# double125/MADTP

Hardware: AMD Instinct MI355X
Metric: images/sec forward, BLIP-base NLVR2 p=0.5 b64; pruned-token index match (higher is better)
Workload: dtype bf16

## Files before the change

madtp_amd/csrc/gemm_device.h:

```cpp
#pragma once
#include "common.h"
#include <type_traits>

namespace {


constexpr int ROWB = 128;
constexpr int NTHREADS = 256;

struct GemmArgs {
    const char* A; const char* W; const float* bias; const float* residual; void* C;
    int M, N, K, lda, ldw, ldc, ldr, act, ntm, ntn, dbg, fast_epi, splitk, ngrp;
    const char* A2; const char* W2; const float* bias2; void* C2; int pair;
    float out_scale;
    float acc_scale;
    float acc_scale2;
    float* sk_ws; int* sk_tick; int sk;
    int desc;
    int* range_flag;
    const int32_t* m_dev; int m_mul;
};
struct F16P { unsigned short bits; };

struct F16S {};
__device__ __forceinline__ bf16x8 x3_scale_lo(bf16x8 q) {
    const f16x8 v = __builtin_bit_cast(f16x8, q) * (_Float16)(1.0f / F16S_LO_SCALE);
    return __builtin_bit_cast(bf16x8, v);
}
template <bool F16>
__device__ __forceinline__ f32x4 mfma_16x16x32(bf16x8 a, bf16x8 b, f32x4 c) {
    if constexpr (F16)
        return __builtin_amdgcn_mfma_f32_16x16x32_f16(__builtin_bit_cast(f16x8, a), __builtin_bit_cast(f16x8, b), c, 0, 0, 0);
    else
        return __builtin_amdgcn_mfma_f32_16x16x32_bf16(a, b, c, 0, 0, 0);
}
constexpr int OM_F32 = 0, OM_BF16 = 1, OM_F16S = 2, OM_F16 = 3;

__device__ __forceinline__ float apply_act(float v, int act) {
    switch (act) {
        case MADTP_ACT_GELU_ERF: return 0.5f * v * (1.0f + erff(v * 0.70710678118654752440f));
        case MADTP_ACT_QUICK_GELU: return v / (1.0f + expf(-1.702f * v));
        case MADTP_ACT_RELU: return fmaxf(v, 0.0f);
        default: return v;
    }
}

template <bool PERM>
__device__ __forceinline__ int swz_key(int r) { return PERM ? (((r >> 1) & 1) | (((r >> 3) & 3) << 1)) : (r & 7); }

__device__ __forceinline__ void xcd_tiles(int T, int xcd, int& t0, int& nt) {
    t0 = (int)(((long)xcd * T) >> 3);
    nt = (int)(((long)(xcd + 1) * T) >> 3) - t0;
}

__device__ __forceinline__ void tile_mn(const GemmArgs& g, int t, int& tm, int& tn) {
    if (g.ngrp == 0) { tm = t / g.ntn; tn = t % g.ntn; return; }
    const int per = g.ntm * g.ngrp;
    const int grp = t / per, r = t - grp * per;
    const int gw = min(g.ngrp, g.ntn - grp * g.ngrp);
    tm = r / gw; tn = grp * g.ngrp + (r - tm * gw);
}

template <int NQ>
__device__ __forceinline__ void stage_tile_desc(const char* base, unsigned bytes, const unsigned* roff, int soff, char* lds) {
    const __amdgpu_buffer_rsrc_t rs = __builtin_amdgcn_make_buffer_rsrc((void*)base, 0, bytes, 0x00020000);
#pragma unroll
    for (int q = 0; q < NQ; ++q) __builtin_amdgcn_raw_ptr_buffer_load_lds(rs, LDS_PTR(lds + q * 1024), 16, roff[q], soff, 0, 0);
}

template <int ESZ, int ROWS, bool PERM = false>
__device__ __forceinline__ void stage_tile(const char* base, int row0, int max_row, int ld_elems, int kbyte0,
                                           char* lds_tile, int wave, int lane, int tile_row0 = 0) {
    const int sub = lane >> 3;
#pragma unroll
    for (int q = 0; q < ROWS / 32; ++q) {
        const int grp = wave * (ROWS / 32) + q;
        const int chunk = (lane & 7) ^ swz_key<PERM>(tile_row0 + grp * 8 + sub);
        int row = row0 + grp * 8 + sub;
        row = row < max_row ? row : max_row;
        const char* src = base + ((size_t)row * ld_elems) * ESZ + kbyte0 + chunk * 16;
        __builtin_amdgcn_global_load_lds(GLOBAL_PTR(src), LDS_PTR(lds_tile + grp * 1024), 16, 0, 0);
    }
}

template <int N> __device__ __forceinline__ void wait_vmcnt() { asm volatile("s_waitcnt vmcnt(%0)" ::"n"(N) : "memory"); }

__device__ __forceinline__ float gelu_fast(float v) {
    constexpr float L2E = 1.4426950408889634f;
    const float x2 = fminf(v * v, 25.0f);
    float p = fmaf(x2, 7.03033581e-04f * L2E, -7.40112921e-02f * L2E);
    p = fmaf(x2, p, -1.59501577f * L2E);
    const float e = __builtin_amdgcn_exp2f(v * p);
    return v * __builtin_amdgcn_rcpf(1.0f + e);
}

template <bool LP_OUT, int ACT>
__device__ __forceinline__ float epi_act(float v) {
    if constexpr (ACT == MADTP_ACT_GELU_ERF) return LP_OUT ? gelu_fast(v) : 0.5f * v * (1.0f + erff(v * 0.70710678118654752440f));
    else if constexpr (ACT == MADTP_ACT_QUICK_GELU)
        return LP_OUT ? v * __builtin_amdgcn_rcpf(1.0f + __builtin_amdgcn_exp2f(-1.702f * 1.4426950408889634f * v))
                      : v / (1.0f + expf(-1.702f * v));
    else if constexpr (ACT == MADTP_ACT_RELU) return fmaxf(v, 0.0f);
    else return v;
}

template <bool LP_OUT>
__host__ __device__ __forceinline__ constexpr int wfrag_row(int j, int rho) {
    return LP_OUT ? 32 * (j >> 1) + 8 * (rho >> 2) + 4 * (j & 1) + (rho & 3) : 16 * j + rho;
}

template <int OM, int ACT, bool HAS_RES, int FM, int FN, int BM, int BN, bool FAST_ONLY = false, int RM = 1, int RN = 1>
__device__ __forceinline__ void epilogue(const GemmArgs& g, const f32x4 (&acc)[FM][FN], const f32x4 (&res)[RM][RN],
                                         int m0, int n0, int wr, int wc, int l16, int grp4, size_t c_off) {
    constexpr bool LP_OUT = OM != OM_F32;
    constexpr bool FAST_ACT = OM == OM_BF16 || OM == OM_F16;
    const bool c_bf16 = g.ldc < 0;
    const int ldc = c_bf16 ? -g.ldc : g.ldc;
            const int col_w = n0 + wc * (BN / 2);
            if (FAST_ONLY || g.fast_epi) {
                constexpr int NJ = LP_OUT ? FN / 2 : FN;
                constexpr int NV = LP_OUT ? 2 : 1;
                constexpr int CSZ = LP_OUT ? 2 : 4;
                constexpr bool RES_PREF = !LP_OUT && RM == FM;
                float range_mx = 0.f;
                const int row_t = m0 + wr * (BM / 2);
                const int rows_valid = max(min(g.M - row_t, BM / 2), 0);
                const unsigned long long cb = (unsigned long long)((char*)g.C + (c_off + (size_t)((g.dbg & 8) ? (row_t & 127) : row_t) * ldc) * CSZ);
                const unsigned cb_lo = __builtin_amdgcn_readfirstlane((unsigned)cb);
                const unsigned cb_hi = __builtin_amdgcn_readfirstlane((unsigned)(cb >> 32));
                const __amdgpu_buffer_rsrc_t crsrc = __builtin_amdgcn_make_buffer_rsrc(
                    (void*)(((unsigned long long)cb_hi << 32) | cb_lo), 0,
                    __builtin_amdgcn_readfirstlane(rows_valid * ldc * CSZ), 0x00020000);
                int colv[NJ];
                bool cok[NJ];
                f32x4 bv[NJ][NV];
#pragma unroll
                for (int jv = 0; jv < NJ; ++jv) {
                    colv[jv] = col_w + (LP_OUT ? 32 * jv + 8 * grp4 : 16 * jv + 4 * grp4);
                    cok[jv] = colv[jv] < g.N;
#pragma unroll
                    for (int u = 0; u < NV; ++u) bv[jv][u] = (f32x4){0.f, 0.f, 0.f, 0.f};
                }
                if (g.bias) {
#pragma unroll
                    for (int jv = 0; jv < NJ; ++jv)
#pragma unroll
                        for (int u = 0; u < NV; ++u) bv[jv][u] = *(const f32x4*)(g.bias + (cok[jv] ? colv[jv] : 0) + 4 * u);
                }
                constexpr bool RES_LOAD = HAS_RES && !RES_PREF;
                constexpr int IC = RES_LOAD ? (FM > 2 ? FM / 2 : FM) : FM;
                f32x4 rv[RES_LOAD ? IC : 1][RES_LOAD ? NJ : 1][NV];
#pragma unroll
                for (int i0 = 0; i0 < FM; i0 += IC) {
                    if constexpr (RES_LOAD) {
#pragma unroll
                        for (int ii = 0; ii < IC; ++ii) {
                            const int row = min(row_t + l16 + 16 * (i0 + ii), g.M - 1);
#pragma unroll
                            for (int jv = 0; jv < NJ; ++jv) {
                                const float* rp = g.residual + (size_t)row * g.ldr + (cok[jv] ? colv[jv] : 0);
#pragma unroll
                                for (int u = 0; u < NV; ++u) rv[ii][jv][u] = *(const f32x4*)(rp + 4 * u);
                            }
                        }
                    }
                    if (RES_LOAD || i0 == 0) {
                        __builtin_amdgcn_sched_barrier(0);
                        __builtin_amdgcn_s_waitcnt(0x0F70);
                        __builtin_amdgcn_sched_barrier(0);
                    }
#pragma unroll
                    for (int ii = 0; ii < IC; ++ii) {
                        const int i = i0 + ii;
#pragma unroll
                        for (int jv = 0; jv < NJ; ++jv) {
                            f32x4 v[NV];
#pragma unroll
                            for (int u = 0; u < NV; ++u) {
#pragma unroll
                                for (int e = 0; e < 4; ++e)
                                    v[u][e] = epi_act<FAST_ACT, ACT>(fmaf(acc[i][NV * jv + u][e], g.acc_scale, bv[jv][u][e])) * g.out_scale;
                                if constexpr (RES_PREF && HAS_RES) v[u] += res[i][jv];
                                if constexpr (RES_LOAD) v[u] += rv[ii][jv][u];
                            }
                            const unsigned off = cok[jv] ? (unsigned)((16 * i + l16) * ldc + colv[jv]) * CSZ : 0x80000000u;
                            u32x4 bits;
                            if constexpr (OM == OM_F16S) {
                                u32x4 lo_bits;
                                split_f16x8(v[0], v[1], bits, lo_bits);
                                __builtin_amdgcn_raw_buffer_store_b128(lo_bits, crsrc, cok[jv] ? off + (unsigned)g.N * 2u : off, 0, 0);
                                range_mx = f16_range_acc(f16_range_acc(range_mx, v[0]), v[1]);
                            } else if constexpr (OM == OM_BF16) bits = __builtin_bit_cast(u32x4, pack_bf16x8(v[0], v[1]));
                            else if constexpr (OM == OM_F16) {
                                bits = __builtin_bit_cast(u32x4, pack_f16x8(v[0], v[1]));
                            }
                            else bits = __builtin_bit_cast(u32x4, v[0]);
                            __builtin_amdgcn_raw_buffer_store_b128(bits, crsrc, off, 0, 0);
                        }
                    }
                }
                if constexpr (OM == OM_F16S) f16_range_raise(g.range_flag, !(range_mx < 65520.0f));
            } else if constexpr (!FAST_ONLY) {
#pragma unroll
                for (int j = 0; j < FN; ++j)
#pragma unroll
                    for (int r = 0; r < 4; ++r) {
                        const int col = col_w + wfrag_row<LP_OUT>(j, 4 * grp4 + r);
                        if (col >= g.N) continue;
                        const float bv = g.bias ? g.bias[col] : 0.0f;
#pragma unroll
                        for (int i = 0; i < FM; ++i) {
                            const int row = m0 + wr * (BM / 2) + i * 16 + l16;
                            if (row >= g.M) continue;
                            float v = epi_act<FAST_ACT, ACT>(fmaf(acc[i][j][r], g.acc_scale, bv)) * g.out_scale;
                            if (g.residual) v += g.residual[(size_t)row * g.ldr + col];
                            const size_t ci = c_off + (size_t)row * ldc + col;
                            if constexpr (OM == OM_F16S) {
                                const _Float16 h = (_Float16)v;
                                ((_Float16*)g.C)[ci] = h;
                                ((_Float16*)g.C)[ci + g.N] = (_Float16)((v - (float)h) * F16S_LO_SCALE);
                                f16_range_raise(g.range_flag, f16_range_bad(v));
                            } else if constexpr (OM == OM_F16) {
                                ((_Float16*)g.C)[ci] = (_Float16)v;
                                f16_range_raise(g.range_flag, f16_range_bad(v));
                            } else if (c_bf16) ((bf16_t*)g.C)[ci] = f32_to_bf16(v);
                            else ((float*)g.C)[ci] = v;
                        }
                    }
            }
}

}
```

madtp_amd/csrc/gemm_pp.hip:

```cpp
#include "gemm_device.h"
#include <stdlib.h>

template <int OM, int MODE, int FA = 4, int ABL = 0, bool SPLITK = false>
__global__ __launch_bounds__(512, 2) void gemm_pp_kernel(GemmArgs g) {
    static_assert(FA == 4 || FA == 3, "256- or 192-row tiles");
    constexpr bool X3 = MODE == 2, F16 = MODE != 0;
    constexpr bool LP_OUT = OM != OM_F32;
    constexpr int BM = 64 * FA, BN = 256, HT = 128 * ROWB;
    extern __shared__ __attribute__((aligned(16))) char smem[];

    const int xcd = blockIdx.x & 7, lb = blockIdx.x >> 3, gl = gridDim.x >> 3;
    const int S = SPLITK ? g.splitk : 1;
    int t0, nslots;
    xcd_tiles(g.ntm * g.ntn * S, xcd, t0, nslots);
    if (lb >= nslots) return;

    const int tid = threadIdx.x, lane = tid & 63;
    const int wave = __builtin_amdgcn_readfirstlane(tid >> 6);
    const int wr = wave >> 2, wc = wave & 3;
    const int nkp = g.K / 64;
    const int nks = __builtin_amdgcn_readfirstlane(nkp / S);

    constexpr int WJ1 = (wfrag_row<LP_OUT>(1, 0) - wfrag_row<LP_OUT>(0, 0)) * ROWB;
    const char* ab[2][2];
    const char* wb[2][2];
    auto frag_bases = [&]() {
        int ln = lane;
        asm volatile("" : "+v"(ln));
        const int l16 = ln & 15, grp4 = ln >> 4;
        const int ra0 = wr * 64 + l16, rw0 = wc * 32 + wfrag_row<LP_OUT>(0, l16);
        const int a_rd = ra0 * ROWB + ((grp4 ^ (l16 & 7)) << 4);
        const int w_rd = rw0 * ROWB + ((grp4 ^ swz_key<LP_OUT>(rw0)) << 4);
        ab[0][0] = smem + a_rd; ab[0][1] = smem + (a_rd ^ 64); ab[1][0] = smem + 65536 + a_rd; ab[1][1] = smem + 65536 + (a_rd ^ 64);
        wb[0][0] = smem + w_rd; wb[0][1] = smem + (w_rd ^ 64); wb[1][0] = smem + 65536 + w_rd; wb[1][1] = smem + 65536 + (w_rd ^ 64);
    };
    frag_bases();

    const int npad = ((g.N + 127) / 128) * 128;
    const __amdgpu_buffer_rsrc_t rs_a = __builtin_amdgcn_make_buffer_rsrc((void*)g.A, 0, (unsigned)((size_t)g.M * g.lda * 2), 0x00020000);
    const __amdgpu_buffer_rsrc_t rs_w = __builtin_amdgcn_make_buffer_rsrc((void*)g.W, 0, (unsigned)((size_t)npad * g.ldw * 2), 0x00020000);
    unsigned va[2][2], vw[2][2];
    int is_slot = lb, is_koff = 0, is_kend = nkp * ROWB;
    const int plane_b = g.K * 2;
    int is_s = 0;
    int is_offa = 0, is_offw = X3 ? plane_b : 0;
    auto tile_offsets = [&]() {
        int tm, tn;
        tile_mn(g, S > 1 ? __builtin_amdgcn_readfirstlane((t0 + is_slot) / S) : t0 + is_slot, tm, tn);
        const unsigned lda2 = (unsigned)g.lda * 2u, ldw2 = (unsigned)g.ldw * 2u;
        int ln = lane;
        asm volatile("" : "+v"(ln));
        const int sub8 = ln >> 3, pos = ln & 7;
#pragma unroll
        for (int q = 0; q < 2; ++q) {
            const int R = (2 * wave + q) * 8 + sub8;
            const unsigned ca = (unsigned)((pos ^ (R & 7)) << 4), cw = (unsigned)((pos ^ swz_key<LP_OUT>(R)) << 4);
            const unsigned rowa = (unsigned)(tm * BM + (R >> 6) * (32 * FA) + (R & 63)), roww = (unsigned)(tn * BN + (R >> 5) * 64 + (R & 31));
            const bool a_ok = FA == 4 || (R & 63) < 16 * FA;
            va[0][q] = a_ok ? rowa * lda2 + ca : 0x80000000u;
            va[1][q] = a_ok ? (rowa + 16u * FA) * lda2 + ca : 0x80000000u;
            vw[0][q] = roww * ldw2 + cw;
            vw[1][q] = (roww + 32u) * ldw2 + cw;
        }
    };
    tile_offsets();
    auto unit_krange = [&]() {
        if (S > 1) {
            const int u = t0 + is_slot, sp = __builtin_amdgcn_readfirstlane(u - (u / S) * S);
            is_koff = sp * nks * ROWB;
            is_kend = is_koff + nks * ROWB;
        } else {
            is_koff = 0;
        }
    };
    unit_krange();
    is_offa = is_koff; is_offw = is_koff + (X3 ? plane_b : 0);
    bool steady = false;
#define PP_ISSUE(RS, V, SLOT, OFF)                                                                                \
    if (!(ABL & 1) || !steady) {                                                                                  \
        char* d__ = smem + (SLOT) * HT + wave * 2048;                                                             \
        __builtin_amdgcn_raw_ptr_buffer_load_lds(RS, LDS_PTR(d__), 16, V[0], OFF, 0, 0);                           \
        __builtin_amdgcn_raw_ptr_buffer_load_lds(RS, LDS_PTR(d__ + 1024), 16, V[1], OFF, 0, 0);                    \
    }
#define PP_ISSUE_A(V, SLOT) PP_ISSUE(rs_a, V, SLOT, is_offa)
#define PP_ISSUE_W(V, SLOT) PP_ISSUE(rs_w, V, SLOT, is_offw)
#define PP_NEXT_SLAB()                                                                         \
    do {                                                                                       \
        if (!X3 || ++is_s == 3) {                                                              \
            is_s = 0;                                                                          \
            is_koff += ROWB;                                                                   \
            if (is_koff == is_kend) { is_slot += gl; tile_offsets(); unit_krange(); }          \
        }                                                                                      \
        is_offa = is_koff + ((X3 && is_s == 2) ? plane_b : 0);                                 \
        is_offw = is_koff + ((X3 && is_s == 0) ? plane_b : 0);                                 \
    } while (0)

    f32x4 acc[2 * FA][4];
    bf16x8 a0[FA][2], a1[FA][2], b0[2][2], b1[2][2];
    const f32x4 zero4 = (f32x4){0.f, 0.f, 0.f, 0.f};
    f32x4 res[1][1];
#define PP_FENCE() __builtin_amdgcn_sched_barrier(0)
#define PP_READ_A(R, P, IDX)                                                                   \
    if (!(ABL & 4) || !steady)                                                                 \
    _Pragma("unroll") for (int i = 0; i < FA; ++i) {                                           \
        R[i][0] = *(const bf16x8*)(ab[P][0] + (IDX) * HT + i * 16 * ROWB);                     \
        R[i][1] = *(const bf16x8*)(ab[P][1] + (IDX) * HT + i * 16 * ROWB);                     \
    }
#define PP_READ_W(R, P, IDX)                                                                   \
    if (!(ABL & 4) || !steady)                                                                 \
    _Pragma("unroll") for (int j = 0; j < 2; ++j) {                                            \
        R[j][0] = *(const bf16x8*)(wb[P][0] + (IDX) * HT + j * WJ1);                           \
        R[j][1] = *(const bf16x8*)(wb[P][1] + (IDX) * HT + j * WJ1);                           \
    }
#define PP_MFMA(RA, RW, SA, SB)                                                                \
    if (!(ABL & 2))                                                                            \
    _Pragma("unroll") for (int ks = 0; ks < 2; ++ks)                                           \
        _Pragma("unroll") for (int i = 0; i < FA; ++i)                                         \
            _Pragma("unroll") for (int j = 0; j < 2; ++j)                                      \
                acc[(SA) * FA + i][(SB) * 2 + j] = mfma_16x16x32<F16>(RW[j][ks], RA[i][ks], acc[(SA) * FA + i][(SB) * 2 + j]);
#define PP_SCALE_W(R, ON)                                                                      \
    if constexpr (X3 && (ON))                                                                  \
    _Pragma("unroll") for (int j = 0; j < 2; ++j) { R[j][0] = x3_scale_lo(R[j][0]); R[j][1] = x3_scale_lo(R[j][1]); }
#define PP_PHASE(READS, ISSUE, PRE, MFMAS)                                                     \
    {                                                                                          \
        READS                                                                                  \
        PP_FENCE();                                                                            \
        if constexpr (!(ABL & 8)) { ISSUE }                                                    \
        PP_FENCE();                                                                            \
        wait_vmcnt<(ABL & 8) ? 8 : 10>();                                                      \
        PP_FENCE();                                                                            \
        __builtin_amdgcn_s_barrier();                                                          \
        PP_FENCE();                                                                            \
        if constexpr ((ABL & 8) != 0) { ISSUE }                                                \
        PP_FENCE();                                                                            \
        __builtin_amdgcn_s_waitcnt(0xC07F);                                    \
        PP_FENCE();                                                                            \
        PRE                                                                                    \
        PP_FENCE();                                                                            \
        if constexpr (!(ABL & 16)) __builtin_amdgcn_s_setprio(1);                              \
        MFMAS                                                                                  \
        if constexpr (!(ABL & 16)) __builtin_amdgcn_s_setprio(0);                              \
        PP_FENCE();                                                                            \
        __builtin_amdgcn_s_barrier();                                                          \
        PP_FENCE();                                                                            \
    }
#define PP_SLAB(P, SC)                                                                                                              \
    PP_PHASE(PP_READ_A(a0, P, 1), PP_ISSUE_W(vw[1], 4 * ((P) ^ 1) + 3); PP_NEXT_SLAB();, PP_SCALE_W(b0, SC), PP_MFMA(a0, b0, 0, 0))   \
    PP_PHASE(PP_READ_A(a1, P, 2), PP_ISSUE_W(vw[0], 4 * (P) + 0);, , PP_MFMA(a1, b0, 1, 0))                                          \
    PP_PHASE(PP_READ_W(b1, P, 3), PP_ISSUE_A(va[0], 4 * (P) + 1);, PP_SCALE_W(b1, SC), PP_MFMA(a1, b1, 1, 1))                        \
    PP_PHASE(PP_READ_W(b0, (P) ^ 1, 0), PP_ISSUE_A(va[1], 4 * (P) + 2);, , PP_MFMA(a0, b1, 0, 1))

    PP_ISSUE_W(vw[0], 0); PP_ISSUE_A(va[0], 1); PP_ISSUE_A(va[1], 2); PP_ISSUE_W(vw[1], 3);
    PP_NEXT_SLAB();
    PP_ISSUE_W(vw[0], 4); PP_ISSUE_A(va[0], 5); PP_ISSUE_A(va[1], 6);
    PP_FENCE();
    wait_vmcnt<10>();
    __builtin_amdgcn_s_barrier();
    PP_FENCE();

    for (int slot = lb; slot < nslots; slot += gl) {
        if (wr == 1) __builtin_amdgcn_s_barrier();
        PP_FENCE();
        if (slot != lb) { frag_bases(); tile_offsets(); }
        PP_READ_W(b0, 0, 0)
        PP_FENCE();
        __builtin_amdgcn_s_waitcnt(0xC07F);
        PP_FENCE();
#pragma unroll
        for (int i = 0; i < 2 * FA; ++i)
#pragma unroll
            for (int j = 0; j < 4; ++j) acc[i][j] = zero4;
        for (int kt = 0; kt < nks; kt += 2) {
            if constexpr (X3) {
                PP_SLAB(0, false)
                PP_SLAB(1, false)
                PP_SLAB(0, true)
                PP_SLAB(1, false)
                PP_SLAB(0, false)
                PP_SLAB(1, true)
            } else {
                PP_SLAB(0, false)
                PP_SLAB(1, false)
            }
            steady = true;
        }
        if (wr == 0) __builtin_amdgcn_s_barrier();
        PP_FENCE();
        int ctm, ctn;
        const int cu = t0 + slot, ct = S > 1 ? __builtin_amdgcn_readfirstlane(cu / S) : cu;
        tile_mn(g, ct, ctm, ctn);
        const size_t c_off = S > 1 ? (size_t)(cu - ct * S) * g.M * (size_t)(g.ldc < 0 ? -g.ldc : g.ldc) : 0;
        const int m0 = ctm * BM, n0 = ctn * BN + (wc >> 1) * 128;
        int lne = lane;
        asm volatile("" : "+v"(lne));
        const int l16e = lne & 15, grp4e = lne >> 4;
#define EPI(ACT)                                                                                                  \
    if constexpr (LP_OUT) {                                                                                       \
        epilogue<OM, ACT, false, 2 * FA, 4, BM, 128>(g, acc, res, m0, n0, wr, wc & 1, l16e, grp4e, c_off);             \
    } else {                                                                                                      \
        if (g.residual) epilogue<OM, ACT, true, 2 * FA, 4, BM, 128>(g, acc, res, m0, n0, wr, wc & 1, l16e, grp4e, c_off); \
        else epilogue<OM, ACT, false, 2 * FA, 4, BM, 128>(g, acc, res, m0, n0, wr, wc & 1, l16e, grp4e, c_off);        \
    }
        switch (g.act) {
            case MADTP_ACT_GELU_ERF: EPI(MADTP_ACT_GELU_ERF) break;
            case MADTP_ACT_QUICK_GELU: EPI(MADTP_ACT_QUICK_GELU) break;
            case MADTP_ACT_RELU: EPI(MADTP_ACT_RELU) break;
            default: EPI(MADTP_ACT_NONE) break;
        }
#undef EPI
    }
    wait_vmcnt<0>();
#undef PP_SLAB
#undef PP_PHASE
#undef PP_SCALE_W
#undef PP_ISSUE_A
#undef PP_ISSUE_W
#undef PP_MFMA
#undef PP_READ_W
#undef PP_READ_A
#undef PP_FENCE
#undef PP_NEXT_SLAB
#undef PP_ISSUE
}

__attribute__((visibility("hidden"))) int madtp_gemm_pp_launch(const void* args, int om, int mode, int rows, int grid, void* stream) {
    const GemmArgs& g = *(const GemmArgs*)args;
    hipStream_t s = (hipStream_t)stream;
    const size_t lds = (size_t)8 * 128 * ROWB;
    static const int abl = env_int("MADTP_PP_ABLATE", 0);
#define PP_LAUNCH(OM_, MODE_, FA_, ABL_)                                                                        \
    do {                                                                                                        \
        MADTP_ENSURE_MAX_LDS((gemm_pp_kernel<OM_, MODE_, FA_, ABL_>), lds);                                      \
        hipLaunchKernelGGL((gemm_pp_kernel<OM_, MODE_, FA_, ABL_>), dim3(grid), dim3(512), lds, s, g);           \
    } while (0)
#define PP_ROWS(OM_, MODE_)                                                                                     \
    do { if (rows == 192) PP_LAUNCH(OM_, MODE_, 3, 0); else PP_LAUNCH(OM_, MODE_, 4, 0); } while (0)
    if (rows != 256 && rows != 192) return MADTP_E_BADARG;
    if (g.splitk > 1) {
        if (mode != 2 || om != OM_F32 || rows != 256 || g.bias || g.residual || g.act != MADTP_ACT_NONE) return MADTP_E_DTYPE;
        MADTP_ENSURE_MAX_LDS((gemm_pp_kernel<OM_F32, 2, 4, 0, true>), lds);
        hipLaunchKernelGGL((gemm_pp_kernel<OM_F32, 2, 4, 0, true>), dim3(grid), dim3(512), lds, s, g);
        return 0;
    }
    if (mode == 2) {
        if (om == OM_F16S) PP_ROWS(OM_F16S, 2); else if (om == OM_F32) PP_ROWS(OM_F32, 2); else return MADTP_E_DTYPE;
    } else if (mode == 1) {
        if (om == OM_F16) PP_ROWS(OM_F16, 1); else if (om == OM_F32) PP_ROWS(OM_F32, 1); else return MADTP_E_DTYPE;
    } else if (om == OM_BF16) {
        switch (rows == 256 ? abl : 0) {
#ifdef MADTP_PP_ABLATIONS
            case 1: PP_LAUNCH(OM_BF16, 0, 4, 1); break;
            case 2: PP_LAUNCH(OM_BF16, 0, 4, 2); break;
            case 3: PP_LAUNCH(OM_BF16, 0, 4, 3); break;
            case 4: PP_LAUNCH(OM_BF16, 0, 4, 4); break;
            case 5: PP_LAUNCH(OM_BF16, 0, 4, 5); break;
            case 6: PP_LAUNCH(OM_BF16, 0, 4, 6); break;
            case 8: PP_LAUNCH(OM_BF16, 0, 4, 8); break;
            case 16: PP_LAUNCH(OM_BF16, 0, 4, 16); break;
#endif
            default: PP_ROWS(OM_BF16, 0); break;
        }
    } else if (om == OM_F32) {
        PP_ROWS(OM_F32, 0);
    } else {
        return MADTP_E_DTYPE;
    }
#undef PP_ROWS
#undef PP_LAUNCH
    return 0;
}
```

Baseline: 26700.

## Overlap GEMM epilogue quadrants with next tile's mainloop in ping-pong kernel

Adds a quadrant-boundary path to the ping-pong GEMM. Each 2x2 quadrant of the accumulator is retired through buffer stores interleaved into the final and first MFMA phases, and the last quadrant is deferred into the next tile's first phase. Bias and residual loads are prefetched during the tail phases. The aim is to hide epilogue store latency behind MFMA work instead of leaving a serialized epilogue per tile. In exchange it adds register pressure, hand-tuned vmcnt wait counts, and a more complex schedule, and it applies only to plain outputs with no activation.

Result: no change. 26560 (-0.5%).

```diff
diff --git a/madtp_amd/csrc/gemm_device.h b/madtp_amd/csrc/gemm_device.h
--- a/madtp_amd/csrc/gemm_device.h
+++ b/madtp_amd/csrc/gemm_device.h
@@ -230,4 +230,107 @@
             }
 }
 
-}
+struct QuadTile {
+    unsigned c_lo, c_hi, c_bytes;
+    unsigned r_lo, r_hi, r_bytes;
+    int col_w;
+};
+constexpr int quad_stores(bool lp_out, int fi) { return lp_out ? fi : 2 * fi; }
+
+__device__ __forceinline__ __amdgpu_buffer_rsrc_t quad_rsrc(unsigned lo, unsigned hi, unsigned bytes) {
+    return __builtin_amdgcn_make_buffer_rsrc((void*)(((unsigned long long)hi << 32) | lo), 0, bytes, 0x00020000);
+}
+
+template <int OM, bool HAS_RES, int BM>
+__device__ __forceinline__ QuadTile quad_tile(const GemmArgs& g, int m0, int col_w, int wr) {
+    constexpr int CSZ = OM != OM_F32 ? 2 : 4;
+    const int ldc = g.ldc < 0 ? -g.ldc : g.ldc;
+    const int row_t = m0 + wr * (BM / 2);
+    const int rows_valid = max(min(g.M - row_t, BM / 2), 0);
+    const unsigned long long cb = (unsigned long long)((char*)g.C + (size_t)row_t * ldc * CSZ);
+    const unsigned long long rb = HAS_RES ? (unsigned long long)(g.residual + (size_t)row_t * g.ldr) : 0ull;
+    QuadTile t;
+    t.c_lo = __builtin_amdgcn_readfirstlane((unsigned)cb);
+    t.c_hi = __builtin_amdgcn_readfirstlane((unsigned)(cb >> 32));
+    t.c_bytes = __builtin_amdgcn_readfirstlane((unsigned)(rows_valid * ldc * CSZ));
+    t.r_lo = __builtin_amdgcn_readfirstlane((unsigned)rb);
+    t.r_hi = __builtin_amdgcn_readfirstlane((unsigned)(rb >> 32));
+    t.r_bytes = HAS_RES ? __builtin_amdgcn_readfirstlane((unsigned)(rows_valid * g.ldr * 4)) : 0u;
+    t.col_w = __builtin_amdgcn_readfirstlane(col_w);
+    return t;
+}
+__device__ __forceinline__ QuadTile quad_tile_none() { return QuadTile{0u, 0u, 0u, 0u, 0u, 0u, 0}; }
+
+template <bool LP_OUT>
+__device__ __forceinline__ int quad_col(const QuadTile& t, int sb, int jq, int grp4) {
+    return t.col_w + (LP_OUT ? 32 * sb + 8 * grp4 : 16 * (2 * sb + jq) + 4 * grp4);
+}
+
+template <int OM, int SB>
+__device__ __forceinline__ void quad_bias(const GemmArgs& g, const QuadTile& t, int lane, u32x4 (&bv)[2]) {
+    constexpr bool LP_OUT = OM != OM_F32;
+    int ln = lane;
+    asm volatile("" : "+v"(ln));
+    const int grp4 = ln >> 4;
+    const __amdgpu_buffer_rsrc_t brs = __builtin_amdgcn_make_buffer_rsrc((void*)g.bias, 0, g.bias ? (unsigned)g.N * 4u : 0u, 0x00020000);
+#pragma unroll
+    for (int u = 0; u < 2; ++u) {
+        const int col = LP_OUT ? quad_col<true>(t, SB, 0, grp4) + 4 * u : quad_col<false>(t, SB, u, grp4);
+        bv[u] = __builtin_amdgcn_raw_buffer_load_b128(brs, col < g.N ? (unsigned)col * 4u : 0x80000000u, 0, 0);
+    }
+}
+
+template <int FI, int SA, int SB>
+__device__ __forceinline__ void quad_residual(const GemmArgs& g, const QuadTile& t, int lane, u32x4 (&rv)[FI][2]) {
+    int ln = lane;
+    asm volatile("" : "+v"(ln));
+    const int l16 = ln & 15, grp4 = ln >> 4;
+    const __amdgpu_buffer_rsrc_t rrs = quad_rsrc(t.r_lo, t.r_hi, t.r_bytes);
+#pragma unroll
+    for (int i = 0; i < FI; ++i)
+#pragma unroll
+        for (int jq = 0; jq < 2; ++jq) {
+            const int col = quad_col<false>(t, SB, jq, grp4);
+            const unsigned off = col < g.N ? (unsigned)((16 * (SA * FI + i) + l16) * g.ldr + col) * 4u : 0x80000000u;
+            rv[i][jq] = __builtin_amdgcn_raw_buffer_load_b128(rrs, off, 0, 0);
+        }
+}
+
+template <int OM, int ACT, bool HAS_RES, int FI, int SA, int SB>
+__device__ __forceinline__ void quad_retire(const GemmArgs& g, const QuadTile& t, const f32x4 (&acc)[2 * FI][4], int lane,
+                                            const u32x4 (&bv)[2], const u32x4 (&rv)[HAS_RES ? FI : 1][2]) {
+    static_assert(OM == OM_F32 || OM == OM_BF16 || OM == OM_F16, "plain outputs only");
+    static_assert(!HAS_RES || OM == OM_F32, "the residual is f32, with the f32 output");
+    constexpr bool LP_OUT = OM != OM_F32;
+    constexpr int CSZ = LP_OUT ? 2 : 4;
+    int ln = lane;
+    asm volatile("" : "+v"(ln));
+    const int l16 = ln & 15, grp4 = ln >> 4;
+    const int ldc = g.ldc < 0 ? -g.ldc : g.ldc;
+    const __amdgpu_buffer_rsrc_t crs = quad_rsrc(t.c_lo, t.c_hi, t.c_bytes);
+#pragma unroll
+    for (int i = 0; i < FI; ++i) {
+        const int fr = SA * FI + i;
+#pragma unroll
+        for (int jq = 0; jq < (LP_OUT ? 1 : 2); ++jq) {
+            f32x4 v[LP_OUT ? 2 : 1];
+#pragma unroll
+            for (int u = 0; u < (LP_OUT ? 2 : 1); ++u) {
+                const f32x4 b = __builtin_bit_cast(f32x4, bv[LP_OUT ? u : jq]);
+#pragma unroll
+                for (int e = 0; e < 4; ++e)
+                    v[u][e] = epi_act<LP_OUT, ACT>(fmaf(acc[fr][2 * SB + (LP_OUT ? u : jq)][e], g.acc_scale, b[e])) * g.out_scale;
+                if constexpr (HAS_RES) v[u] += __builtin_bit_cast(f32x4, rv[i][jq]);
+            }
+            const int col = quad_col<LP_OUT>(t, SB, jq, grp4);
+            const unsigned off = col < g.N ? (unsigned)((16 * fr + l16) * ldc + col) * CSZ : 0x80000000u;
+            u32x4 bits;
+            if constexpr (OM == OM_BF16) bits = __builtin_bit_cast(u32x4, pack_bf16x8(v[0], v[1]));
+            else if constexpr (OM == OM_F16) bits = __builtin_bit_cast(u32x4, pack_f16x8(v[0], v[1]));
+            else bits = __builtin_bit_cast(u32x4, v[0]);
+            __builtin_amdgcn_raw_buffer_store_b128(bits, crs, off, 0, 0);
+        }
+    }
+}
+
+}
diff --git a/madtp_amd/csrc/gemm_pp.hip b/madtp_amd/csrc/gemm_pp.hip
--- a/madtp_amd/csrc/gemm_pp.hip
+++ b/madtp_amd/csrc/gemm_pp.hip
@@ -1,10 +1,20 @@
 #include "gemm_device.h"
 #include <stdlib.h>
 
-template <int OM, int MODE, int FA = 4, int ABL = 0, bool SPLITK = false>
+constexpr int pp_quad_wait(bool res, int ns, int fa, int p) {
+    const bool bias_f0 = !res && fa == 3;
+    const int nl = res ? 2 + 2 * fa : 0;
+    const int e[8] = {res ? nl : (bias_f0 ? 0 : 4), ns + nl, ns + nl, ns + nl, ns + (bias_f0 ? 4 : 0), 0, 0, 0};
+    int x = 10;
+    for (int q = p > 4 ? p - 4 : 0; q <= p; ++q) x += e[q];
+    return x < 63 ? x : 63;
+}
+template <int OM, int MODE, int FA = 4, int ABL = 0, bool SPLITK = false, int QACT = -1, bool QRES = false>
 __global__ __launch_bounds__(512, 2) void gemm_pp_kernel(GemmArgs g) {
     static_assert(FA == 4 || FA == 3, "256- or 192-row tiles");
     constexpr bool X3 = MODE == 2, F16 = MODE != 0;
+    constexpr bool QB = QACT >= 0;
+    static_assert(!QB || (!X3 && !SPLITK && ABL == 0 && (OM == OM_F32 || !QRES)), "quadrant boundary: plain operands and outputs");
     constexpr bool LP_OUT = OM != OM_F32;
     constexpr int BM = 64 * FA, BN = 256, HT = 128 * ROWB;
     extern __shared__ __attribute__((aligned(16))) char smem[];
@@ -150,6 +160,42 @@
     PP_PHASE(PP_READ_W(b1, P, 3), PP_ISSUE_A(va[0], 4 * (P) + 1);, PP_SCALE_W(b1, SC), PP_MFMA(a1, b1, 1, 1))                        \
     PP_PHASE(PP_READ_W(b0, (P) ^ 1, 0), PP_ISSUE_A(va[1], 4 * (P) + 2);, , PP_MFMA(a0, b1, 0, 1))
 
+#define PP_MFMA_Z(RA, RW, SA, SB)                                                              \
+    _Pragma("unroll") for (int ks = 0; ks < 2; ++ks)                                           \
+        _Pragma("unroll") for (int i = 0; i < FA; ++i)                                         \
+            _Pragma("unroll") for (int j = 0; j < 2; ++j)                                      \
+                acc[(SA) * FA + i][(SB) * 2 + j] =                                             \
+                    mfma_16x16x32<F16>(RW[j][ks], RA[i][ks], ks == 0 ? zero4 : acc[(SA) * FA + i][(SB) * 2 + j]);
+#define PP_QPHASE(P, EARLY, READS, RETIRE, PREF, ISSUE, MFMAS)                                 \
+    {                                                                                          \
+        EARLY                                                                                  \
+        PP_FENCE();                                                                            \
+        READS                                                                                  \
+        PP_FENCE();                                                                            \
+        RETIRE                                                                                 \
+        PP_FENCE();                                                                            \
+        PREF                                                                                   \
+        PP_FENCE();                                                                            \
+        ISSUE                                                                                  \
+        PP_FENCE();                                                                            \
+        wait_vmcnt<pp_quad_wait(QRES, quad_stores(LP_OUT, FA), FA, P)>();                      \
+        PP_FENCE();                                                                            \
+        __builtin_amdgcn_s_barrier();                                                          \
+        PP_FENCE();                                                                            \
+        __builtin_amdgcn_s_waitcnt(0xC07F);                                    \
+        PP_FENCE();                                                                            \
+        __builtin_amdgcn_s_setprio(1);                                                         \
+        MFMAS                                                                                  \
+        __builtin_amdgcn_s_setprio(0);                                                         \
+        PP_FENCE();                                                                            \
+        __builtin_amdgcn_s_barrier();                                                          \
+        PP_FENCE();                                                                            \
+    }
+#define PP_QRETIRE(T, SA, SB) quad_retire<OM, QB ? QACT : 0, QRES, FA, SA, SB>(g, T, acc, lane, qbv[SB], qrv);
+#define PP_QRETIRE_IF(C, T, SA, SB) if constexpr (C) { PP_QRETIRE(T, SA, SB) }
+#define PP_QBIAS_IF(C, T, SB) if constexpr (C) { quad_bias<OM, SB>(g, T, lane, qbv[SB]); }
+#define PP_QRES(T, SA, SB) if constexpr (QRES) { quad_residual<FA, SA, SB>(g, T, lane, qrv); }
+
     PP_ISSUE_W(vw[0], 0); PP_ISSUE_A(va[0], 1); PP_ISSUE_A(va[1], 2); PP_ISSUE_W(vw[1], 3);
     PP_NEXT_SLAB();
     PP_ISSUE_W(vw[0], 4); PP_ISSUE_A(va[0], 5); PP_ISSUE_A(va[1], 6);
@@ -158,6 +204,54 @@
     __builtin_amdgcn_s_barrier();
     PP_FENCE();
 
+    if constexpr (QB) {
+        constexpr bool EARLY = QRES;
+        constexpr bool BIAS_F0 = !QRES && FA == 3;
+        u32x4 qbv[2][2];
+        u32x4 qrv[QRES ? FA : 1][2];
+        qbv[0][0] = qbv[0][1] = qbv[1][0] = qbv[1][1] = (u32x4){0u, 0u, 0u, 0u};
+#pragma unroll
+        for (int i = 0; i < (QRES ? FA : 1); ++i) qrv[i][0] = qrv[i][1] = (u32x4){0u, 0u, 0u, 0u};
+#pragma unroll
+        for (int i = 0; i < 2 * FA; ++i)
+#pragma unroll
+            for (int j = 0; j < 4; ++j) acc[i][j] = zero4;
+        QuadTile pend = quad_tile_none();
+        if (wr == 1) __builtin_amdgcn_s_barrier();
+        PP_FENCE();
+        PP_READ_W(b0, 0, 0)
+        PP_FENCE();
+        __builtin_amdgcn_s_waitcnt(0xC07F);
+        PP_FENCE();
+        for (int slot = lb; slot < nslots; slot += gl) {
+            int ctm, ctn;
+            tile_mn(g, t0 + slot, ctm, ctn);
+            const QuadTile cur = quad_tile<OM, QRES, BM>(g, ctm * BM, ctn * BN + wc * 64, wr);
+            PP_QPHASE(4, PP_QRETIRE_IF(EARLY, pend, 0, 1), PP_READ_A(a0, 0, 1), PP_QRETIRE_IF(!EARLY, pend, 0, 1),
+                      PP_QBIAS_IF(BIAS_F0, cur, 0) PP_QBIAS_IF(BIAS_F0, cur, 1),
+                      PP_ISSUE_W(vw[1], 7); PP_NEXT_SLAB();, PP_MFMA_Z(a0, b0, 0, 0))
+            PP_QPHASE(5, , PP_READ_A(a1, 0, 2), , , PP_ISSUE_W(vw[0], 0);, PP_MFMA_Z(a1, b0, 1, 0))
+            PP_QPHASE(6, , PP_READ_W(b1, 0, 3), , , PP_ISSUE_A(va[0], 1);, PP_MFMA_Z(a1, b1, 1, 1))
+            PP_QPHASE(7, , PP_READ_W(b0, 1, 0), , , PP_ISSUE_A(va[1], 2);, PP_MFMA_Z(a0, b1, 0, 1))
+            for (int kt = 2; kt < nks; kt += 2) {
+                PP_SLAB(1, false)
+                PP_SLAB(0, false)
+            }
+            PP_QPHASE(0, , PP_READ_A(a0, 1, 1), , PP_QBIAS_IF(!BIAS_F0, cur, 0) PP_QBIAS_IF(!BIAS_F0 && !QRES, cur, 1) PP_QRES(cur, 0, 0),
+                      PP_ISSUE_W(vw[1], 3); PP_NEXT_SLAB();, PP_MFMA(a0, b0, 0, 0))
+            PP_QPHASE(1, PP_QRETIRE_IF(EARLY, cur, 0, 0), PP_READ_A(a1, 1, 2), PP_QRETIRE_IF(!EARLY, cur, 0, 0),
+                      PP_QBIAS_IF(QRES, cur, 0) PP_QRES(cur, 1, 0), PP_ISSUE_W(vw[0], 4);, PP_MFMA(a1, b0, 1, 0))
+            PP_QPHASE(2, PP_QRETIRE_IF(EARLY, cur, 1, 0), PP_READ_W(b1, 1, 3), PP_QRETIRE_IF(!EARLY, cur, 1, 0),
+                      PP_QBIAS_IF(QRES, cur, 1) PP_QRES(cur, 1, 1), PP_ISSUE_A(va[0], 5);, PP_MFMA(a1, b1, 1, 1))
+            PP_QPHASE(3, PP_QRETIRE_IF(EARLY, cur, 1, 1), PP_READ_W(b0, 0, 0), PP_QRETIRE_IF(!EARLY, cur, 1, 1),
+                      PP_QBIAS_IF(QRES, cur, 1) PP_QRES(cur, 0, 1), PP_ISSUE_A(va[1], 6);, PP_MFMA(a0, b1, 0, 1))
+            pend = cur;
+        }
+        PP_QRETIRE(pend, 0, 1)
+        PP_FENCE();
+        if (wr == 0) __builtin_amdgcn_s_barrier();
+        PP_FENCE();
+    } else
     for (int slot = lb; slot < nslots; slot += gl) {
         if (wr == 1) __builtin_amdgcn_s_barrier();
         PP_FENCE();
@@ -210,6 +304,12 @@
 #undef EPI
     }
     wait_vmcnt<0>();
+#undef PP_QRES
+#undef PP_QBIAS_IF
+#undef PP_QRETIRE_IF
+#undef PP_QRETIRE
+#undef PP_QPHASE
+#undef PP_MFMA_Z
 #undef PP_SLAB
 #undef PP_PHASE
 #undef PP_SCALE_W
@@ -242,6 +342,27 @@
         hipLaunchKernelGGL((gemm_pp_kernel<OM_F32, 2, 4, 0, true>), dim3(grid), dim3(512), lds, s, g);
         return 0;
     }
+    static const int quad = env_int("MADTP_PP_EPI", 1);
+    const bool res = om == OM_F32 && g.residual;
+    if (quad && mode != 2 && g.fast_epi && g.dbg == 0 && g.act == MADTP_ACT_NONE &&
+        (!res || (size_t)g.ldr * 128 * 4 < ((size_t)1 << 31)) &&
+        ((mode == 0 && (om == OM_BF16 || om == OM_F32)) || (mode == 1 && (om == OM_F16 || om == OM_F32))) &&
+        (rows == 192 || abl == 0)) {
+#define PP_QLAUNCH(OM_, MODE_, FA_, RES_)                                                                                       \
+    do {                                                                                                                        \
+        MADTP_ENSURE_MAX_LDS((gemm_pp_kernel<OM_, MODE_, FA_, 0, false, MADTP_ACT_NONE, RES_>), lds);                            \
+        hipLaunchKernelGGL((gemm_pp_kernel<OM_, MODE_, FA_, 0, false, MADTP_ACT_NONE, RES_>), dim3(grid), dim3(512), lds, s, g); \
+    } while (0)
+#define PP_QROWS(OM_, MODE_, RES_)                                                                                              \
+    do { if (rows == 192) PP_QLAUNCH(OM_, MODE_, 3, RES_); else PP_QLAUNCH(OM_, MODE_, 4, RES_); } while (0)
+#define PP_QF32(MODE_) do { if (res) PP_QROWS(OM_F32, MODE_, true); else PP_QROWS(OM_F32, MODE_, false); } while (0)
+        if (mode == 0) { if (om == OM_BF16) PP_QROWS(OM_BF16, 0, false); else PP_QF32(0); }
+        else { if (om == OM_F16) PP_QROWS(OM_F16, 1, false); else PP_QF32(1); }
+#undef PP_QF32
+#undef PP_QROWS
+#undef PP_QLAUNCH
+        return 0;
+    }
     if (mode == 2) {
         if (om == OM_F16S) PP_ROWS(OM_F16S, 2); else if (om == OM_F32) PP_ROWS(OM_F32, 2); else return MADTP_E_DTYPE;
     } else if (mode == 1) {
```
